# drtconway/zotmer

Measured on AMD Instinct MI355X. Metric: Gk-mers/sec kmerize k=25 on synthetic 150bp FASTQ; achieved HBM GB/s fraction, higher is better.
Workload: dtype u64

## Files before the change

### include/zotk.h

```cpp
#ifndef ZOTK_H
#define ZOTK_H

#include <stdint.h>

#ifdef __cplusplus
extern "C" {
#endif

#define ZK_OK 0
#define ZK_EINVAL (-1)
#define ZK_ENOMEM (-2)
#define ZK_EHIP (-3)
#define ZK_ENOSPC (-4)
#define ZK_EOVERFLOW (-5)
#define ZK_EINTERNAL (-6)
#define ZK_ERANGE (-7)

typedef struct zk_ctx zk_ctx;

zk_ctx* zk_create(int device, uint64_t workspace_bytes);
void zk_destroy(zk_ctx* ctx);
const char* zk_last_error(zk_ctx* ctx);
int zk_set_stream(zk_ctx* ctx, void* hip_stream);
void* zk_get_stream(zk_ctx* ctx);
// ... 8 lines not shown
int zk_copy(zk_ctx* ctx, void* d_dst, const void* d_src, uint64_t bytes);
int zk_host_alloc(zk_ctx* ctx, uint64_t bytes, void** ptr);
int zk_host_free(zk_ctx* ctx, void* ptr);
int zk_upload_async(zk_ctx* ctx, void* d_dst, const void* src, uint64_t bytes);

#define ZK_TUNE_SORT_VARIANT 1
#define ZK_TUNE_PAIRS_VARIANT 2
#define ZK_TUNE_SHORT_SORT 3
#define ZK_TUNE_XCD_GROUP 5
#define ZK_TUNE_SIDE_DIV 4
#define ZK_TUNE_EARLY_COLLAPSE 7
#define ZK_TUNE_PACKED_PAIRS 8
#define ZK_TUNE_WIDE_TILES 9
#define ZK_TUNE_STREAM_PASS 10
#define ZK_TUNE_STREAM_RANGES 11
#define ZK_TUNE_TAG_WORDS 12
#define ZK_TUNE_DEDUPE_VARIANT 13
#define ZK_TUNE_DEDUPE_LIMIT 14
#define ZK_TUNE_DEDUPE_BITS 15
#define ZK_TUNE_COMM_CHUNK 6
#define ZK_TUNE_TAG_PASS 17
#define ZK_TUNE_KWAY 18
#define ZK_TUNE_TILE_SORT 19
#define ZK_TUNE_COMM_SELF_LOOP 16
int zk_tune(zk_ctx* ctx, int what, int value);

#define ZK_PROF_HIST_STREAM 1
#define ZK_PROF_HIST_ARRAY 2
#define ZK_PROF_PASS_STREAM 3
#define ZK_PROF_PASS_KEYS 4
#define ZK_PROF_PASS_PAIRS 5
#define ZK_PROF_RLE 6
#define ZK_PROF_UNION 7
#define ZK_PROF_SELECT 8
#define ZK_PROF_MIRROR 9
#define ZK_PROF_INTERSECT 10
#define ZK_PROF_COUNT_HIST 11
#define ZK_PROF_PASS_PACKED 12
#define ZK_PROF_SAMPLE 13
#define ZK_PROF_TILE_SORT 14
#define ZK_PROF_CAPTURE_HITS 15
int zk_debug_buffer(zk_ctx* ctx, void* d_buf);
int zk_profile(zk_ctx* ctx, int enable);
int zk_profile_read(zk_ctx* ctx, int tag, uint64_t* launches, double* total_ms, uint64_t* algorithmic_bytes);


// ... 156 lines not shown
```

### zotmer_amd/csrc/context.hip

```cpp
#include <stdarg.h>
#include <string.h>

#include "internal.hpp"
#include <vector>

namespace zk {

int fail(zk_ctx* c, int code, const char* fmt, ...) {
    char buf[512];
    va_list ap;
    va_start(ap, fmt);
    vsnprintf(buf, sizeof buf, fmt, ap);
    va_end(ap);
    if (c) c->last_error = buf;
    return code;
}

void arena_reset(zk_ctx* c) { c->arena_off = 0; }

int arena_alloc(zk_ctx* c, uint64_t bytes, void** p) {
    const uint64_t need = (bytes + 255) & ~255ull;
    if (c->arena_off + need > c->arena_size) {
        if (c->arena_off != 0)
            return fail(c, ZK_ENOMEM, "workspace too small: %llu bytes in use, %llu more needed, %llu reserved (call zk_reserve)",
// ... 273 lines not shown
    if (what == ZK_TUNE_PAIRS_VARIANT) { c->pairs_variant = value; return ZK_OK; }
    if (what == ZK_TUNE_SHORT_SORT) { c->short_sort = value; return ZK_OK; }
    if (what == ZK_TUNE_SIDE_DIV) { c->side_div = value; return ZK_OK; }
    if (what == ZK_TUNE_WIDE_TILES) { c->wide_tiles = value ? 1 : 0; return ZK_OK; }
    if (what == ZK_TUNE_PACKED_PAIRS) { c->packed_pairs = value ? 1 : 0; return ZK_OK; }
    if (what == ZK_TUNE_EARLY_COLLAPSE) { c->early_collapse = value < 0 ? 0 : (value > 3 ? 3 : value); return ZK_OK; }
    if (what == ZK_TUNE_COMM_SELF_LOOP) { c->comm_self_loop = value ? 1 : 0; return ZK_OK; }
    if (what == ZK_TUNE_COMM_CHUNK) { c->comm_chunk_bytes = value > 0 ? (uint64_t)value : 0; return ZK_OK; }
    if (what == ZK_TUNE_STREAM_PASS) {
#ifdef ZK_PHASES
        c->stream_pass = value < 0 ? 0 : value;
#else
        if (value < 0 || value > 3) return fail(c, ZK_EINVAL, "stream pass variant %d (0, 1, 2 or 3)", value);
        c->stream_pass = value;
#endif
        return ZK_OK;
    }
    if (what == ZK_TUNE_TAG_WORDS) { c->tag_words = value < 0 ? 0 : (value > 2 ? 2 : value); return ZK_OK; }
    if (what == ZK_TUNE_DEDUPE_VARIANT) { c->dedupe_variant = value < 0 ? -1 : (value & 3); return ZK_OK; }
    if (what == ZK_TUNE_KWAY) { c->kway = value < 0 ? 0 : (value > 2 ? 2 : value); return ZK_OK; }
    if (what == ZK_TUNE_TILE_SORT) { c->tile_sort = value ? 1 : 0; return ZK_OK; }
    if (what == ZK_TUNE_TAG_PASS) { c->tag_pass = value ? 1 : 0; return ZK_OK; }
    if (what == ZK_TUNE_DEDUPE_BITS) { c->dedupe_bits = value < 0 ? 0 : value; return ZK_OK; }
    if (what == ZK_TUNE_DEDUPE_LIMIT) { c->dedupe_limit = value < 1 ? 1 : (value > 65536 ? 65536 : value); return ZK_OK; }
    if (what == ZK_TUNE_STREAM_RANGES) { c->stream_ranges = value < 0 ? 0 : (value > 4096 ? 4096 : value); return ZK_OK; }
    if (what == ZK_TUNE_XCD_GROUP) {
        if (value < 0 || value > 32 || (value & (value - 1))) return fail(c, ZK_EINVAL, "xcd group must be 0 or a power of two <= 32");
        c->xcd_group = value;
        return ZK_OK;
    }
    return fail(c, ZK_EINVAL, "unknown tuning knob %d", what);
}

int zk_debug_buffer(zk_ctx* c, void* d_buf) {
    if (!c) return ZK_EINVAL;
    enter(c);
    c->dbg = (u64*)d_buf;
    return ZK_OK;
}

int zk_profile(zk_ctx* c, int enable) {
    if (!c) return ZK_EINVAL;
    enter(c);
    ZK_HIP(c, hipStreamSynchronize(c->stream));
    for (auto& r : c->prof) { (void)hipEventDestroy(r.a); (void)hipEventDestroy(r.b); }
    c->prof.clear();
// ... 91 lines not shown
```

### zotmer_amd/csrc/internal.hpp

```cpp
#pragma once
#include <hip/hip_runtime.h>
#include <stdint.h>
#include <stdio.h>
#include <string>
#include <vector>

#include "../../include/zotk.h"
#include "common.hpp"

struct zk_ctx {
    int device = 0;
    hipStream_t stream = nullptr;
    bool own_stream = false;
    int num_cus = 256;
    int sort_variant = 3;
    int short_sort = 0;
    int packed_pairs = 1;
    int wide_tiles = 1;
    int early_collapse = 1;
    int side_div = 8;
    int pairs_variant = 7;
    int stream_pass = 1;
    int tag_words = 2;
    int dedupe_variant = 0;
    int dedupe_limit = 65536;
    int tag_pass = 0;
    int kway = 1;
    int tile_sort = 1;
    int dedupe_bits = 0;
    int stream_ranges = 0;

    char* arena = nullptr;
    uint64_t arena_size = 0;
    uint64_t arena_off = 0;

    char* aux = nullptr;
    uint64_t aux_size = 0;

    u64* status = nullptr;
    uint64_t status_words = 0;
    unsigned short* part16 = nullptr;
    uint64_t part16_words = 0;
    u32 epoch = 0;
    u32* d_ticket = nullptr;
    u32* d_xticket = nullptr;
    int num_xcd = 1;
    int xcd_group = 0;
    u32 ticket_base = 0;

    u32* d_err = nullptr;
    u64* d_scalars = nullptr;
    u64* h_scalars = nullptr;
// ... 63 lines not shown
struct StreamSample { int shift; uint64_t value; double max_ratio; uint64_t seen = 0, distinct = 0; bool want_distinct = false; };
struct StreamTags { bool written = false; u64* cuts = nullptr; uint32_t blocks = 0; };
struct StreamSrc { const u8* stream; uint64_t n_bytes; int K; int mode; int lo_bit; int hi_bit = 0; StreamSample* sample = nullptr;
                   StreamTags* tags = nullptr; };
int sort_rbits(zk_ctx* c);
PassPlan sort_plan_upper(zk_ctx* c, int key_bits, int lo_bit);
struct MirrorHist { int passes; int shift[4]; int bits[4]; u64* raw; };
int sort_first_bits(zk_ctx* c, int key_bits, int lo_bit);
struct DedupeResult {
    uint64_t n_out = 0;
    uint32_t flags = 0;
    uint32_t n_big = 0;
    u64 *cuts = nullptr, *nwords = nullptr, *incl = nullptr, *big = nullptr, *work = nullptr;
    u32* sub = nullptr;
    uint32_t chunks = 0;
    int pack = 0;
};
int dedupe_pass(zk_ctx* c, const u64* keys, uint64_t n, int key_bits, int b, int pack, u64* work, uint64_t cap, DedupeResult* r,
                uint64_t* n_in = nullptr, uint64_t max_chunks = 0, const u32* tags = nullptr, const u64* tag_cuts = nullptr);
int expand_tags(zk_ctx* c, const u32* tags, const u64* cuts, uint32_t blocks, int tag_bits, u64* keys_out, uint64_t first_block = 0, uint64_t n_blocks = 0);
int dedupe_finish(zk_ctx* c, const DedupeResult& r, u64* out_k, u32* out_c, u64* out_m = nullptr, int K = 0, int gbases = 0,
                  u64** mirror_hist = nullptr, int* mirror_group_bits = nullptr, bool packed_out = false);
int sort_keys_upper_counted(zk_ctx* c, u64* keys, u64* alt, uint64_t n, int key_bits, int lo_bit, u64* counted, u64** result);
int collapse_pass(zk_ctx* c, const u64* keys, uint64_t n, int shift, int bits, int pack, u64* out, uint64_t cap, uint64_t* n_out,
                  uint64_t max_tiles = 0);
int sort_stream(zk_ctx* c, const StreamSrc& src, u64* buf_a, u64* buf_b, uint64_t cap, uint64_t* n_keys,
                uint64_t acgt[4], u64** result);
struct StreamRows { u32* rows = nullptr; u64* offs = nullptr; u32 ranges = 0, radix = 0; u32* gcodes = nullptr; u16* gvalid = nullptr;
                    u32 strands = 1;
                    bool wide = false; };
int stream_hist(zk_ctx* c, const u8* stream, uint64_t n_bytes, int K, int mode, const PassPlan& plan, u64* ghist, u32 gstride,
                u64* d_acgt, u64* d_n, u64* rec_info, u64* sample, u32 sample_cap, int sample_shift, u64 sample_value, u32* sample_n,
                void* image_room, uint64_t image_room_bytes, StreamRows* out);
struct StreamPlanes { u16* dig; int shift, bits; };
int stream_pass0(zk_ctx* c, uint64_t n_bytes, int K, int mode, int shift, int bits, const u64* ghist0, const StreamRows& rows,
                 uint64_t first_nl, bool uniform, u64* kout, uint64_t n, int variant, const StreamPlanes* planes = nullptr);
int stream_pass1(zk_ctx* c, const u32* tags, const u16* dig, uint64_t n, const u64* ghist0, uint32_t radix0, int bits1, u32* tout, u64* cuts);
int tile_sort_top_bits(uint64_t n, int key_bits, int rbits);
int tile_sort(zk_ctx* c, u64* keys, u32* vals, uint64_t n, int key_bits, int top, bool* declined);
int tile_sort_count(zk_ctx* c, const u64* keys, uint64_t n, int key_bits, int top, u64* uniq, u32* counts, uint64_t cap, uint64_t* n_unique,
                    bool* declined);
int trim(zk_ctx* c, const u64* keys, const void* cnts, int cbits, uint64_t n, u64 lo, u64 hi, u64* ok, void* oc,
         uint64_t cap, uint64_t* n_out);
int project_dedupe(zk_ctx* c, const u64* keys, uint64_t n, int shift, u64* out, uint64_t cap, uint64_t* n_out);
int subsample(zk_ctx* c, const u64* keys, uint64_t n, u64 seed, double p, u64* out, uint64_t cap, uint64_t* n_out);
int sample_pairs(zk_ctx* c, const u64* keys, const u64* cnts, uint64_t n, u64 seed, double p, u64* ok, u64* oc, uint64_t cap,
// ... 38 lines not shown
```

### zotmer_amd/csrc/pipeline.hip

```cpp
#include <string.h>

#include <vector>

#include "internal.hpp"

namespace zk {

__global__ void mirror_kernel(const u64* __restrict__ c, const u32* __restrict__ n, u64 m, int K, u64* __restrict__ r,
                              u32* __restrict__ v) {
    for (u64 i = (u64)blockIdx.x * blockDim.x + threadIdx.x; i < m; i += (u64)gridDim.x * blockDim.x) {
        r[i] = revcomp(K, c[i]);
        v[i] = n[i];
    }
}

constexpr int MIRROR_GROUP_BITS = 18;
constexpr int MIRROR_GROUP_BASES = MIRROR_GROUP_BITS / 2;

__global__ void mirror_bounds_kernel(const u64* __restrict__ c, u64 n, int K, int gbits, u64* __restrict__ start) {
    const u32 g = blockIdx.x * blockDim.x + threadIdx.x;
    if (g > (1u << gbits)) return;
    const u64 want = (u64)g << (2 * K - gbits);
    u64 lo = 0, hi = n;
    if (g == (1u << gbits)) lo = n;
// ... 298 lines not shown
    u64* other = (sorted == buf_a) ? buf_b : buf_a;
    u32* cnt = (u32*)other;
    uint64_t uc = 0;
    bool in_aux = false;
    uint64_t max_count = 0;
    bool have_max = false;
    bool canon_packed = false;
    u64 *mwords = nullptr, *malt = nullptr;
    u64* mhist = nullptr;
    int mgroup = MIRROR_GROUP_BITS;
    if (dedupe_bit && n) {
        const int pk = pack_bits_for(K);
        DedupeResult r;
        uint64_t n_in = 0;
        bool done = false;
        const uint64_t nblocks = 1ull << dedupe_bit, per = n / nblocks + 1;
        const u32* tg = stags.written ? (const u32*)sorted : nullptr;
        if (!presampled) ZK_TRY(dedupe_pass(c, sorted, n, 2 * K, dedupe_bit, pk, other, cap_keys, &r, &n_in, (1u << 20) / per + 4, tg, stags.cuts));
        if (presampled || (!(r.flags & 1) && (double)r.n_out <= 0.6 * (double)n_in)) {
            ZK_TRY(dedupe_pass(c, sorted, n, 2 * K, dedupe_bit, pk, other, cap_keys, &r, nullptr, 0, tg, stags.cuts));
            if (!(r.flags & 1)) {
                uc = r.n_out;
                const uint64_t a8 = (8 * uc + 255) & ~255ull, a4 = (4 * uc + 255) & ~255ull;
                char* aux;
                ZK_TRY(aux_require(c, a8 + a4, &aux));
                const bool want_m = !(r.flags & 2) && !canonical_only && c->packed_pairs && dedupe_bit == MIRROR_GROUP_BITS &&
                                    2 * K >= MIRROR_GROUP_BITS + 8;
                ZK_TRY(dedupe_finish(c, r, (u64*)aux, (u32*)(aux + a8), want_m ? sorted : nullptr, K, MIRROR_GROUP_BASES, &mhist, &mgroup, want_m));
                if (want_m) { mwords = sorted; malt = other; canon_packed = true; }
                sorted = (u64*)aux; cnt = (u32*)(aux + a8);
                in_aux = true;
                if (!(r.flags & 2)) { max_count = (1ull << pk) - 1; have_max = true; }
                done = true;
            }
        }
        if (!done) {
            u64* res = nullptr;
            if (tg) {
                ZK_TRY(expand_tags(c, tg, stags.cuts, stags.blocks, 2 * K - dedupe_bit, other));
                u64* t = sorted; sorted = other; other = t;
            }
            ZK_TRY(sort_keys(c, sorted, other, n, 2 * K, &res));
            sorted = res;
            other = (sorted == buf_a) ? buf_b : buf_a;
            cnt = (u32*)other;
        }
        fused_bit = 0;
        collapse_bit = 0;
    }
    if (fused_bit && n) {
// ... 302 lines not shown
```

### zotmer_amd/csrc/tilesort.hip

```cpp
#include "internal.hpp"

#ifdef ZK_PHASES
#define TS_PHASE(k) do { if (a.dbg) { const u32 now__ = (u32)__builtin_amdgcn_s_memtime(); ph[k] += now__ - tlast; tlast = now__; } } while (0)
#else
#define TS_PHASE(k) do { } while (0)
#endif

namespace zk {

constexpr int TS_BLOCK = 512;
constexpr u32 TS_SLACK = 1024;

template <int ITEMS, int GROUPS, bool PAIRS>
struct TileSortSmem {
    static constexpr int CAP = TS_BLOCK * ITEMS;
    alignas(16) u64 keys[CAP];
    u32 vals[PAIRS ? CAP : 1];
    u16 idx[PAIRS ? CAP : 1];
    alignas(16) u32 start[GROUPS + 8];
    u32 wsum[TS_BLOCK / 64];
};
typedef TileSortSmem<14, 4096, false> TileSortKeys;
constexpr int TS_COUNT_ITEMS = 12;
typedef TileSortSmem<10, 2048, true> TileSortPairs;

struct TileSortArgs {
    const u64* kin; u64* kout;
    const u32* vin; u32* vout;
    const u64* bounds;
    u32 tiles;
    int pshift;
};

__global__ void tile_bounds_kernel(const u64* __restrict__ a, u64 n, int pshift, u32 T, u32 S, u32 tiles, u64* __restrict__ bounds,
                                   u32* __restrict__ flag) {
    const u32 t = blockIdx.x * blockDim.x + threadIdx.x;
    if (t > tiles) return;
    if (t == 0) { bounds[0] = 0; return; }
    if (t == tiles) { bounds[tiles] = n; return; }
    const u64 p = (u64)t * T;
    const u64 pre = a[p] >> pshift;
    u64 lo = p - S, hi = p;
    if ((a[lo] >> pshift) == pre) {
        atomicOr(flag, 1u);
        bounds[t] = lo;
        return;
    }
    while (hi - lo > 1) {
        const u64 mid = lo + (hi - lo) / 2;
        if ((a[mid] >> pshift) == pre) hi = mid; else lo = mid;
    }
    bounds[t] = hi;
}

struct TileMap {
    u64 kmin; int sh; u32 scale;
    __device__ __forceinline__ u32 group(u64 key) const {
        const u32 d = (u32)((key - kmin) >> sh);
        return scale ? __umulhi(d, scale) : d;
    }
};

template <int ITEMS, int G, bool PAIRS, class S>
__device__ __forceinline__ TileMap tile_group(S& sm, const u64* kin, const u32* vin, u64 lo, u32 m, int pshift, int tid) {
    constexpr int NW = TS_BLOCK / 64, QPT = G / TS_BLOCK / 4;
    static_assert(QPT == 1 || QPT == 2, "four or eight groups a thread in the scan");
    static_assert(S::CAP <= 8192 && G <= 4096, "group | place << 12 in a word");
    const int lane = tid & 63, wave = __builtin_amdgcn_readfirstlane(tid >> 6);
    const u64* kp = kin + lo;
    u64 k[ITEMS];
    u32 v[PAIRS ? ITEMS : 1];
#pragma unroll
    for (int j = 0; j < ITEMS; j++) {
        const u32 i = (u32)j * TS_BLOCK + tid;
        k[j] = i < m ? kp[i] : ~0ull;
        if constexpr (PAIRS) v[j] = i < m ? vin[lo + i] : 0u;
    }
    const u64 first = kp[0], last = kp[m - 1];
    TileMap tm;
    tm.kmin = (first >> pshift) << pshift;
    const u64 rm1 = (((last >> pshift) - (first >> pshift)) << pshift) | ((1ull << pshift) - 1ull);
    tm.sh = rm1 >> 32 ? 32 - __builtin_clzll(rm1) : 0;
    const u32 rs = (u32)(rm1 >> tm.sh);
    tm.scale = rs < (u32)G ? 0u : (u32)(((u64)G << 32) / ((u64)rs + 1ull));
    {
        uint4* z = reinterpret_cast<uint4*>(sm.start);
#pragma unroll
        for (int q = 0; q < QPT; q++) z[QPT * tid + q] = make_uint4(0, 0, 0, 0);
    }
    __syncthreads();
    u32 gp[ITEMS];
#pragma unroll
    for (int j = 0; j < ITEMS; j++) {
        const u32 i = (u32)j * TS_BLOCK + tid;
        const u32 g = i < m ? tm.group(k[j]) : 0u;
        gp[j] = g;
        if (i < m) gp[j] |= atomicAdd(&sm.start[g], 1u) << 12;
    }
    __syncthreads();
    {
        uint4* z = reinterpret_cast<uint4*>(sm.start);
        uint4 cq[QPT];
        u32 sum = 0;
#pragma unroll
        for (int q = 0; q < QPT; q++) { cq[q] = z[QPT * tid + q]; sum += cq[q].x + cq[q].y + cq[q].z + cq[q].w; }
        const u32 inc = wave_incl_scan_u32(sum);
        if (lane == 63) sm.wsum[wave] = inc;
        __syncthreads();
        u32 run = inc - sum;
#pragma unroll
        for (int w = 0; w < NW; w++) run += w < wave ? sm.wsum[w] : 0u;
#pragma unroll
        for (int q = 0; q < QPT; q++) {
            uint4 sq;
            sq.x = run; run += cq[q].x; sq.y = run; run += cq[q].y; sq.z = run; run += cq[q].z; sq.w = run; run += cq[q].w;
            z[QPT * tid + q] = sq;
        }
        if (tid == 0) sm.start[G] = m;
    }
    __syncthreads();
#pragma unroll
    for (int j = 0; j < ITEMS; j++) {
        const u32 i = (u32)j * TS_BLOCK + tid;
        if (i < m) {
            const u32 p = sm.start[gp[j] & (G - 1)] + (gp[j] >> 12);
            sm.keys[p] = k[j];
            if constexpr (PAIRS) { sm.vals[p] = v[j]; sm.idx[p] = (u16)i; }
        }
    }
    __syncthreads();
    return tm;
}

template <int E, bool PAIRS, class S>
__device__ __forceinline__ void tile_rank(const S& sm, const TileMap& tm, const u32 (&i)[E], u32 m, u64 (&mine)[E], u32 (&place)[E]) {
    constexpr u32 CAP = S::CAP;
    auto before = [&](u64 ko, u32 q, u64 km, u32 at) -> bool {
        if (ko != km) return ko < km;
        if constexpr (PAIRS) return q != at && sm.idx[q] < sm.idx[at];
        else return q < at;
    };
    u32 g0[E], g1[E];
#pragma unroll
    for (int e = 0; e < E; e++) mine[e] = sm.keys[i[e] < m ? i[e] : 0u];
#pragma unroll
    for (int e = 0; e < E; e++) {
        const u32 g = tm.group(mine[e]);
        g0[e] = sm.start[g]; g1[e] = sm.start[g + 1];
    }
    u64 o[E][4];
#pragma unroll
    for (int e = 0; e < E; e++)
#pragma unroll
        for (int r = 0; r < 4; r++) o[e][r] = sm.keys[g0[e] + r < CAP ? g0[e] + r : CAP - 1];
#pragma unroll
    for (int e = 0; e < E; e++) {
        const u32 at = i[e] < m ? i[e] : 0u;
        u32 rank = 0;
#pragma unroll
        for (int r = 0; r < 4; r++) {
            const u32 q = g0[e] + r;
            rank += (q < g1[e] && before(o[e][r], q, mine[e], at)) ? 1u : 0u;
        }
        for (u32 q0 = g0[e] + 4; q0 < g1[e]; q0 += 4) {
            u64 p4[4];
#pragma unroll
            for (int r = 0; r < 4; r++) p4[r] = sm.keys[q0 + r < CAP ? q0 + r : CAP - 1];
#pragma unroll
            for (int r = 0; r < 4; r++) {
                const u32 q = q0 + r;
                rank += (q < g1[e] && before(p4[r], q, mine[e], at)) ? 1u : 0u;
            }
        }
        place[e] = g0[e] + rank;
    }
}

template <int ITEMS, int G, bool PAIRS>
__global__ __launch_bounds__(TS_BLOCK, 2 * TS_BLOCK / 256) void tile_sort_kernel(TileSortArgs a) {
    using S = TileSortSmem<ITEMS, G, PAIRS>;
    constexpr int CAP = S::CAP;
    static_assert(sizeof(S) <= 80 * 1024, "two workgroups per CU");
    __shared__ S sm;
    for (u32 t = blockIdx.x; t < a.tiles; t += gridDim.x) {
        int tid = threadIdx.x;
        asm volatile("" : "+v"(tid));
        const u64 lo = a.bounds[t], hi = a.bounds[t + 1];
        if (hi - lo > (u64)CAP || hi == lo) continue;
        const u32 m = (u32)(hi - lo);
        const TileMap tm = tile_group<ITEMS, G, PAIRS>(sm, a.kin, a.vin, lo, m, a.pshift, tid);
        constexpr int E = 2;
        u64* op = a.kout + lo;
        for (u32 i0 = (u32)tid; i0 < m; i0 += E * TS_BLOCK) {
            u32 i[E], place[E];
            u64 mine[E];
#pragma unroll
            for (int e = 0; e < E; e++) i[e] = i0 + e * TS_BLOCK;
            tile_rank<E, PAIRS>(sm, tm, i, m, mine, place);
// ... 223 lines not shown
```

### zotmer_amd/native.py

```python
import ctypes as C
import os

import numpy as np

_HERE = os.path.dirname(os.path.abspath(__file__))
LIB_PATH = os.environ.get("ZOTK_LIB") or os.path.join(_HERE, "libzotk.so")

ZK_OK, ZK_EINVAL, ZK_ENOMEM, ZK_EHIP, ZK_ENOSPC, ZK_EOVERFLOW, ZK_EINTERNAL, ZK_ERANGE = 0, -1, -2, -3, -4, -5, -6, -7
KMERIZE_CANONICAL, KMERIZE_BOTH, KMERIZE_SUBSAMPLE, KMERIZE_CANONICAL_ONLY = 0, 1, 2, 4
DEFAULT_TAG_WORDS = 2

_ERRNAMES = {-1: "ZK_EINVAL", -2: "ZK_ENOMEM", -3: "ZK_EHIP", -4: "ZK_ENOSPC", -5: "ZK_EOVERFLOW",
             -6: "ZK_EINTERNAL", -7: "ZK_ERANGE"}


class ZotkError(RuntimeError):
    def __init__(self, code, msg):
        super().__init__("%s: %s" % (_ERRNAMES.get(code, code), msg))
        self.code = code


class KmerizeStats(C.Structure):
    _fields_ = [("n_windows", C.c_uint64), ("n_instances", C.c_uint64), ("n_unique", C.c_uint64),
                ("n_canonical", C.c_uint64), ("acgt", C.c_uint64 * 4)]
# ... 275 lines not shown
        cut = C.c_uint64(0)
        self._check(self.lib.zk_last_newline(self.h, text.ptr, int(n), C.byref(cut)))
        return cut.value

    def device_to_file(self, arr, fileno, offset, threads=None):
        self._check(self.lib.zk_device_to_file(self.h, arr.ptr, arr.nbytes, int(fileno), int(offset), threads or self.IO_THREADS))

    def file_to_device(self, fileno, offset, nbytes, dtype=np.uint8, threads=None):
        dt = np.dtype(dtype)
        out = self.empty(nbytes // dt.itemsize, dt)
        self._check(self.lib.zk_file_to_device(self.h, int(fileno), int(offset), int(nbytes), out.ptr, threads or self.IO_THREADS))
        return out

    def upload_stream(self, data):
        a = np.frombuffer(data, dtype=np.uint8) if isinstance(data, (bytes, bytearray, memoryview)) else np.asarray(data, np.uint8)
        return self.upload(a)

    PROF_TAGS = {"hist_stream": 1, "hist_array": 2, "pass_stream": 3, "pass_keys": 4, "pass_pairs": 5, "rle": 6,
                 "union_sum": 7, "select": 8, "mirror": 9, "intersect": 10, "count_hist": 11, "pass_packed": 12, "sample": 13, "tile_sort": 14,
                 "capture_hits": 15}

    def tune(self, sort_variant=None, pairs_variant=None, short_sort=None, side_div=None, xcd_group=None, comm_chunk=None,
             early_collapse=None, packed_pairs=None, wide_tiles=None, stream_pass=None, stream_ranges=None, tag_words=None,
             dedupe_variant=None, dedupe_limit=None, dedupe_bits=None, comm_self_loop=None, tag_pass=None, kway=None, tile_sort=None):
        if tile_sort is not None:
            self._check(self.lib.zk_tune(self.h, 19, int(tile_sort)))
        if kway is not None:
            self._check(self.lib.zk_tune(self.h, 18, int(kway)))
        if tag_pass is not None:
            self._check(self.lib.zk_tune(self.h, 17, int(tag_pass)))
        if comm_self_loop is not None:
            self._check(self.lib.zk_tune(self.h, 16, int(comm_self_loop)))
        if dedupe_bits is not None:
            self._check(self.lib.zk_tune(self.h, 15, int(dedupe_bits)))
        if dedupe_variant is not None:
            self._check(self.lib.zk_tune(self.h, 13, int(dedupe_variant)))
        if dedupe_limit is not None:
            self._check(self.lib.zk_tune(self.h, 14, int(dedupe_limit)))
        if tag_words is not None:
            self._check(self.lib.zk_tune(self.h, 12, int(tag_words)))
        if stream_pass is not None:
            self._check(self.lib.zk_tune(self.h, 10, int(stream_pass)))
        if stream_ranges is not None:
            self._check(self.lib.zk_tune(self.h, 11, int(stream_ranges)))
        if wide_tiles is not None:
            self._check(self.lib.zk_tune(self.h, 9, int(wide_tiles)))
        if packed_pairs is not None:
# ... 389 lines not shown
```

Measured before the change: 155.7.

## Merge canonical and mirrored strands per top-bit block via shared-memory tile union

For odd K with mirror output, a new path builds the reverse-complement mirror words, sorts them by their upper bits, and then merges each of the 2^18 canonical blocks with its matching mirror range inside shared memory. It writes the final keys and counts directly, which is meant to replace the dedupe_finish plus separate union pass. Blocks that are too large or too crowded go to a slower split kernel, and if that also fails the code falls back to the old path. The tile grouping code moves into a shared header so both the tile sort and this new path can use it.

```diff
diff --git a/include/zotk.h b/include/zotk.h
--- a/include/zotk.h
+++ b/include/zotk.h
@@ -54,6 +54,7 @@
 #define ZK_TUNE_TAG_PASS 17
 #define ZK_TUNE_KWAY 18
 #define ZK_TUNE_TILE_SORT 19
+#define ZK_TUNE_STRAND_BLOCKS 20
 #define ZK_TUNE_COMM_SELF_LOOP 16
 int zk_tune(zk_ctx* ctx, int what, int value);
 
diff --git a/zotmer_amd/csrc/context.hip b/zotmer_amd/csrc/context.hip
--- a/zotmer_amd/csrc/context.hip
+++ b/zotmer_amd/csrc/context.hip
@@ -319,6 +319,7 @@
     if (what == ZK_TUNE_TILE_SORT) { c->tile_sort = value ? 1 : 0; return ZK_OK; }
     if (what == ZK_TUNE_TAG_PASS) { c->tag_pass = value ? 1 : 0; return ZK_OK; }
     if (what == ZK_TUNE_DEDUPE_BITS) { c->dedupe_bits = value < 0 ? 0 : value; return ZK_OK; }
+    if (what == ZK_TUNE_STRAND_BLOCKS) { c->strand_blocks = value ? 1 : 0; return ZK_OK; }
     if (what == ZK_TUNE_DEDUPE_LIMIT) { c->dedupe_limit = value < 1 ? 1 : (value > 65536 ? 65536 : value); return ZK_OK; }
     if (what == ZK_TUNE_STREAM_RANGES) { c->stream_ranges = value < 0 ? 0 : (value > 4096 ? 4096 : value); return ZK_OK; }
     if (what == ZK_TUNE_XCD_GROUP) {
diff --git a/zotmer_amd/csrc/internal.hpp b/zotmer_amd/csrc/internal.hpp
--- a/zotmer_amd/csrc/internal.hpp
+++ b/zotmer_amd/csrc/internal.hpp
@@ -28,6 +28,7 @@
     int kway = 1;
     int tile_sort = 1;
     int dedupe_bits = 0;
+    int strand_blocks = 1;
     int stream_ranges = 0;
 
     char* arena = nullptr;
@@ -137,6 +138,8 @@
 int dedupe_finish(zk_ctx* c, const DedupeResult& r, u64* out_k, u32* out_c, u64* out_m = nullptr, int K = 0, int gbases = 0,
                   u64** mirror_hist = nullptr, int* mirror_group_bits = nullptr, bool packed_out = false);
 int sort_keys_upper_counted(zk_ctx* c, u64* keys, u64* alt, uint64_t n, int key_bits, int lo_bit, u64* counted, u64** result);
+int strand_blocks(zk_ctx* c, const DedupeResult& r, u64* keys_buf, uint64_t buf_words, int K, u64* out_k, u32* out_c, uint64_t cap,
+                  uint64_t* n_out);
 int collapse_pass(zk_ctx* c, const u64* keys, uint64_t n, int shift, int bits, int pack, u64* out, uint64_t cap, uint64_t* n_out,
                   uint64_t max_tiles = 0);
 int sort_stream(zk_ctx* c, const StreamSrc& src, u64* buf_a, u64* buf_b, uint64_t cap, uint64_t* n_keys,
diff --git a/zotmer_amd/csrc/pipeline.hip b/zotmer_amd/csrc/pipeline.hip
--- a/zotmer_amd/csrc/pipeline.hip
+++ b/zotmer_amd/csrc/pipeline.hip
@@ -344,10 +344,14 @@
             if (!(r.flags & 1)) {
                 uc = r.n_out;
                 const uint64_t a8 = (8 * uc + 255) & ~255ull, a4 = (4 * uc + 255) & ~255ull;
+                const bool want_m = !(r.flags & 2) && !canonical_only && c->packed_pairs && dedupe_bit == MIRROR_GROUP_BITS &&
+                                    2 * K >= MIRROR_GROUP_BITS + 8;
+                if (want_m && (K & 1) && c->strand_blocks && 2 * a8 <= 8 * cap_keys) {
+                    st->n_canonical = uc;
+                    return strand_blocks(c, r, sorted, cap_keys, K, out_k, out_c, cap, n_out);
+                }
                 char* aux;
                 ZK_TRY(aux_require(c, a8 + a4, &aux));
-                const bool want_m = !(r.flags & 2) && !canonical_only && c->packed_pairs && dedupe_bit == MIRROR_GROUP_BITS &&
-                                    2 * K >= MIRROR_GROUP_BITS + 8;
                 ZK_TRY(dedupe_finish(c, r, (u64*)aux, (u32*)(aux + a8), want_m ? sorted : nullptr, K, MIRROR_GROUP_BASES, &mhist, &mgroup, want_m));
                 if (want_m) { mwords = sorted; malt = other; canon_packed = true; }
                 sorted = (u64*)aux; cnt = (u32*)(aux + a8);
diff --git a/zotmer_amd/csrc/strand_blocks.hip b/zotmer_amd/csrc/strand_blocks.hip
--- /dev/null
+++ b/zotmer_amd/csrc/strand_blocks.hip
@@ -0,0 +1,314 @@
+#include "tile_group.hpp"
+
+namespace zk {
+
+constexpr int SB_ITEMS = 16, SB_GROUPS = 2048;
+constexpr u32 SB_GROUP_MAX = 128;
+typedef TileSortSmem<SB_ITEMS, SB_GROUPS, false> StrandSmem;
+constexpr int SB_BLOCK_BITS = 18;
+
+__global__ __launch_bounds__(256) void strand_mirror_kernel(const u64* __restrict__ in, const u64* __restrict__ cuts, const u64* __restrict__ incl,
+                                                            const u64* __restrict__ nwords, u32 chunks, int pack, int K, u64* __restrict__ out_m,
+                                                            MirrorHist mh) {
+    __shared__ u32 bins[4 * 512];
+    const bool hist = mh.passes > 0;
+    if (hist) {
+        for (int q = threadIdx.x; q < 4 * 512; q += blockDim.x) bins[q] = 0;
+        __syncthreads();
+    }
+    const u64 maxc = (1ull << pack) - 1;
+    for (u32 v = blockIdx.x; v < chunks; v += gridDim.x) {
+        const u64 cnt = nwords[v];
+        const u64 dst0 = incl[v] - cnt;
+        const u64* src = in + cuts[v];
+        for (u64 i0 = threadIdx.x; i0 < cnt; i0 += 4ull * blockDim.x) {
+            u64 w4[4];
+#pragma unroll
+            for (int q = 0; q < 4; q++) {
+                const u64 i = i0 + (u64)q * blockDim.x;
+                w4[q] = i < cnt ? src[i] : 0;
+            }
+#pragma unroll
+            for (int q = 0; q < 4; q++) {
+                const u64 i = i0 + (u64)q * blockDim.x;
+                if (i >= cnt) break;
+                const u64 mw = (revcomp(K, w4[q] >> pack) << pack) | (w4[q] & maxc);
+                out_m[dst0 + i] = mw;
+                if (hist) {
+#pragma unroll
+                    for (int p = 0; p < 4; p++)
+                        if (p < mh.passes) atomicAdd(&bins[p * 512 + ((u32)(mw >> mh.shift[p]) & ((1u << mh.bits[p]) - 1u))], 1u);
+                }
+            }
+        }
+    }
+    if (hist) {
+        __syncthreads();
+        for (int q = threadIdx.x; q < mh.passes * 512; q += blockDim.x)
+            if (bins[q]) atomicAdd(&mh.raw[q], (u64)bins[q]);
+    }
+}
+
+__global__ void strand_starts_kernel(const u64* __restrict__ m, u64 n, int shift, u64* __restrict__ start) {
+    const u32 g = blockIdx.x * blockDim.x + threadIdx.x;
+    if (g > (1u << SB_BLOCK_BITS)) return;
+    u64 lo = 0, hi = n;
+    if (g == (1u << SB_BLOCK_BITS)) lo = n;
+    while (lo < hi) {
+        const u64 mid = (lo + hi) >> 1;
+        if ((m[mid] >> shift) < (u64)g) lo = mid + 1; else hi = mid;
+    }
+    start[g] = lo;
+}
+
+struct StrandArgs {
+    const u64* cw;
+    const u64* cuts; const u64* nwords; const u64* incl;
+    const u64* m;
+    const u64* mstart;
+    u64* ok; u32* oc;
+    int pack;
+    int pshift;
+    u32* n_declined;
+    u32* declined;
+};
+
+__device__ __forceinline__ bool strand_crowded(const StrandSmem& sm, int tid) {
+    static_assert(SB_GROUPS == 4 * TS_BLOCK, "four groups a thread");
+    u32 big = 0;
+#pragma unroll
+    for (int q = 0; q < 4; q++) big |= sm.start[4 * tid + q + 1] - sm.start[4 * tid + q] > SB_GROUP_MAX ? 1u : 0u;
+    return __syncthreads_or((int)big) != 0;
+}
+
+__device__ __forceinline__ void strand_write(const StrandSmem& sm, const TileMap& tm, u32 m, u64* ok, u32* oc, int pack, int tid) {
+    const u64 maxc = (1ull << pack) - 1;
+    constexpr int E = 2;
+    for (u32 i0 = (u32)tid; i0 < m; i0 += E * TS_BLOCK) {
+        u32 i[E], place[E];
+        u64 mine[E];
+#pragma unroll
+        for (int e = 0; e < E; e++) i[e] = i0 + e * TS_BLOCK;
+        tile_rank<E, false>(sm, tm, i, m, mine, place);
+#pragma unroll
+        for (int e = 0; e < E; e++) {
+            if (i[e] >= m) break;
+            ok[place[e]] = mine[e] >> pack;
+            oc[place[e]] = (u32)(mine[e] & maxc);
+        }
+    }
+}
+
+__global__ __launch_bounds__(TS_BLOCK, 2 * TS_BLOCK / 256) void strand_block_union_kernel(StrandArgs a) {
+    using S = StrandSmem;
+    constexpr u32 CAP = S::CAP;
+    static_assert(sizeof(S) <= 80 * 1024, "two workgroups per CU");
+    __shared__ S sm;
+    const u32 b = blockIdx.x;
+    const u64 nc = a.nwords[b], m0 = a.mstart[b], nm = a.mstart[b + 1] - m0;
+    const u64 n = nc + nm;
+    if (n == 0) return;
+    if (n > CAP) {
+        if (threadIdx.x == 0) a.declined[atomicAdd(a.n_declined, 1u)] = b;
+        return;
+    }
+    int tid = threadIdx.x;
+    asm volatile("" : "+v"(tid));
+    const u32 m = (u32)n;
+    const TileMap tm = tile_group<SB_ITEMS, SB_GROUPS, false>(sm, a.cw, nullptr, a.cuts[b], m, a.pshift, tid, a.m, m0, (u32)nc);
+    if (strand_crowded(sm, tid)) {
+        if (tid == 0) a.declined[atomicAdd(a.n_declined, 1u)] = b;
+        return;
+    }
+    const u64 out0 = a.incl[b] - nc + m0;
+    strand_write(sm, tm, m, a.ok + out0, a.oc + out0, a.pack, tid);
+}
+
+constexpr int SB_SPLIT = 256;
+struct StrandBigSmem {
+    StrandSmem t;
+    u64 sp[SB_SPLIT];
+    u32 mcnt[SB_SPLIT + 2];
+    u32 cpos[SB_SPLIT + 2];
+    u32 tile[SB_SPLIT + 2];
+    u32 ntiles, gcount, fail;
+};
+
+__global__ __launch_bounds__(TS_BLOCK) void strand_big_block_kernel(StrandArgs a, u32 n_list, u64* __restrict__ scratch, u32* __restrict__ fail) {
+    using S = StrandBigSmem;
+    constexpr u32 CAP = StrandSmem::CAP, R = SB_SPLIT + 1;
+    __shared__ S sm;
+    u64* gat = scratch + (u64)blockIdx.x * CAP;
+    const int lane = threadIdx.x & 63;
+    for (u32 li = blockIdx.x; li < n_list; li += gridDim.x) {
+        int tid = threadIdx.x;
+        asm volatile("" : "+v"(tid));
+        const u32 b = a.declined[li];
+        const u64 nc = a.nwords[b], m0 = a.mstart[b], nm = a.mstart[b + 1] - m0;
+        const u64* C = a.cw + a.cuts[b];
+        const u64* M = a.m + m0;
+        const u64 bmin = (u64)b << a.pshift, bmax = bmin | ((1ull << a.pshift) - 1ull);
+        const u64 out0 = a.incl[b] - nc + m0;
+        u64* cand = sm.t.keys;
+        if (tid < SB_SPLIT) {
+            const bool one = nm == 0 || nc == 0;
+            const bool fromc = nm == 0 || (nc && tid < SB_SPLIT / 2);
+            const u32 j = one || fromc ? (u32)tid : (u32)tid - SB_SPLIT / 2, per = one ? SB_SPLIT : SB_SPLIT / 2;
+            cand[tid] = fromc ? C[(u64)j * nc / per] : M[(u64)j * nm / per];
+        }
+        if (tid == 0) { sm.fail = 0; sm.gcount = 0; }
+        if (tid < (int)R + 1) sm.mcnt[tid] = 0;
+        __syncthreads();
+        if (tid < SB_SPLIT) {
+            const u64 v = cand[tid];
+            u32 r = 0;
+            for (int q = 0; q < SB_SPLIT; q++) { const u64 o = cand[q]; r += (o < v || (o == v && q < tid)) ? 1u : 0u; }
+            sm.sp[r] = v;
+        }
+        __syncthreads();
+        auto range_of = [&](u64 v) -> u32 {
+            u32 lo = 0, hi = SB_SPLIT;
+            while (lo < hi) { const u32 mid = (lo + hi) >> 1; if (sm.sp[mid] <= v) lo = mid + 1; else hi = mid; }
+            return lo;
+        };
+        for (u64 i = tid; i < nm; i += TS_BLOCK) atomicAdd(&sm.mcnt[range_of(M[i])], 1u);
+        if (tid <= SB_SPLIT) {
+            u32 p = 0;
+            if (tid > 0) {
+                const u64 v = sm.sp[tid - 1];
+                u64 lo = 0, hi = nc;
+                while (lo < hi) { const u64 mid = (lo + hi) >> 1; if (C[mid] < v) lo = mid + 1; else hi = mid; }
+                p = (u32)lo;
+            }
+            sm.cpos[tid] = p;
+        }
+        if (tid == 0) sm.cpos[R] = (u32)nc;
+        __syncthreads();
+        if (tid == 0) {
+            u32 acc = 0, nt = 0, mb = 0;
+            sm.tile[nt++] = 0;
+            for (u32 j = 0; j < R; j++) {
+                const u32 mc = sm.mcnt[j], tot = sm.cpos[j + 1] - sm.cpos[j] + mc;
+                if (tot > CAP) { sm.fail = 1; break; }
+                if (acc + tot > CAP) { sm.tile[nt++] = j; acc = 0; }
+                acc += tot;
+                sm.mcnt[j] = mb;
+                mb += mc;
+            }
+            sm.mcnt[R] = mb;
+            sm.tile[nt] = R;
+            sm.ntiles = nt;
+        }
+        __syncthreads();
+        if (sm.fail) {
+            if (tid == 0) atomicOr(fail, 1u);
+            continue;
+        }
+        const u32 ntiles = sm.ntiles;
+        for (u32 t = 0; t < ntiles; t++) {
+            const u32 ra = sm.tile[t], rb = sm.tile[t + 1];
+            const u64 vlo = ra == 0 ? bmin : sm.sp[ra - 1];
+            const u64 vhi = rb == R ? bmax : sm.sp[rb - 1] - 1;
+            const u32 c_lo = sm.cpos[ra], mc = sm.cpos[rb] - c_lo, mt = sm.mcnt[rb] - sm.mcnt[ra];
+            const u32 m = mc + mt;
+            if (m == 0) continue;
+            if (mt) {
+                for (u64 i0 = 0; i0 < nm; i0 += TS_BLOCK) {
+                    const u64 i = i0 + tid;
+                    const u64 v = i < nm ? M[i] : 0;
+                    const bool in = i < nm && v >= vlo && v <= vhi;
+                    const u64 bal = __ballot(in);
+                    u32 base = 0;
+                    if (lane == 0 && bal) base = atomicAdd(&sm.gcount, (u32)__popcll(bal));
+                    base = (u32)__shfl((int)base, 0, 64);
+                    if (in) gat[base + popc_below(bal)] = v;
+                }
+                __threadfence_block();
+            }
+            __syncthreads();
+            const TileMap tm = tile_group<SB_ITEMS, SB_GROUPS, false>(sm.t, C, nullptr, c_lo, m, a.pshift, tid, gat, 0, mc, true, vlo, vhi);
+            if (strand_crowded(sm.t, tid)) {
+                if (tid == 0) atomicOr(fail, 1u);
+                break;
+            }
+            const u64 o = out0 + c_lo + sm.mcnt[ra];
+            strand_write(sm.t, tm, m, a.ok + o, a.oc + o, a.pack, tid);
+            if (tid == 0) sm.gcount = 0;
+            __syncthreads();
+        }
+        __syncthreads();
+    }
+}
+
+int strand_blocks(zk_ctx* c, const DedupeResult& r, u64* keys_buf, uint64_t buf_words, int K, u64* out_k, u32* out_c, uint64_t cap,
+                  uint64_t* n_out) {
+    *n_out = 0;
+    const uint64_t uc = r.n_out;
+    if (uc == 0) return ZK_OK;
+    if (!(K & 1) || r.n_big || r.chunks != (1u << SB_BLOCK_BITS)) return fail(c, ZK_EINTERNAL, "strand_blocks: K %d, %u big counts, %u blocks", K, r.n_big, r.chunks);
+    const uint64_t a8w = ((8 * uc + 255) & ~255ull) / 8;
+    if (2 * a8w > buf_words) return fail(c, ZK_EINTERNAL, "strand_blocks: %llu words do not fit twice in %llu", (unsigned long long)uc, (unsigned long long)buf_words);
+    if (2 * uc > cap) return fail(c, ZK_ENOSPC, "output holds %llu entries, the table has %llu", (unsigned long long)cap, (unsigned long long)(2 * uc));
+    const int pk = r.pack, key_bits = 2 * K + pk, lo_bit = key_bits - SB_BLOCK_BITS;
+    u64* mw = keys_buf;
+    u64* malt = keys_buf + a8w;
+    MirrorHist mh = {};
+    if (c->sort_variant == 3) {
+        const PassPlan plan = sort_plan_upper(c, key_bits, lo_bit);
+        if (plan.passes <= 4) {
+            ZK_TRY(arena_alloc(c, sizeof(u64) * MAX_PASSES * 512, (void**)&mh.raw));
+            ZK_HIP(c, hipMemsetAsync(mh.raw, 0, sizeof(u64) * MAX_PASSES * 512, c->stream));
+            mh.passes = plan.passes;
+            for (int p = 0; p < plan.passes; p++) { mh.shift[p] = plan.shift[p]; mh.bits[p] = plan.bits[p]; }
+        }
+    }
+    prof_begin(c, ZK_PROF_SELECT, 16 * uc);
+    hipLaunchKernelGGL(strand_mirror_kernel, dim3((u32)c->num_cus * 8), dim3(256), 0, c->stream, r.work, r.cuts, r.incl, r.nwords, r.chunks, pk, K, mw, mh);
+    prof_end(c);
+    ZK_HIP(c, hipGetLastError());
+    u64* sk = nullptr;
+    if (mh.passes) ZK_TRY(sort_keys_upper_counted(c, mw, malt, uc, key_bits, lo_bit, mh.raw, &sk));
+    else ZK_TRY(sort_keys_upper(c, mw, malt, uc, key_bits, lo_bit, &sk));
+    u64* mstart;
+    u32* declined;
+    ZK_TRY(arena_alloc(c, sizeof(u64) * ((1ull << SB_BLOCK_BITS) + 1), (void**)&mstart));
+    ZK_TRY(arena_alloc(c, sizeof(u32) * r.chunks, (void**)&declined));
+    StrandArgs a = {};
+    a.cw = r.work; a.cuts = r.cuts; a.nwords = r.nwords; a.incl = r.incl; a.m = sk; a.mstart = mstart;
+    a.ok = out_k; a.oc = out_c; a.pack = pk; a.pshift = lo_bit;
+    a.n_declined = (u32*)(c->d_scalars + 9);
+    a.declined = declined;
+    u32* fail = (u32*)(c->d_scalars + 9) + 1;
+    prof_begin(c, ZK_PROF_UNION, 8 * 2 * uc + 12 * 2 * uc);
+    hipLaunchKernelGGL(strand_starts_kernel, dim3(((1u << SB_BLOCK_BITS) + 256) / 256), dim3(256), 0, c->stream, sk, (u64)uc, lo_bit, mstart);
+    ZK_HIP(c, hipMemsetAsync(c->d_scalars + 9, 0, sizeof(u64), c->stream));
+    hipLaunchKernelGGL(strand_block_union_kernel, dim3(r.chunks), dim3(TS_BLOCK), 0, c->stream, a);
+    prof_end(c);
+    ZK_HIP(c, hipGetLastError());
+    ZK_HIP(c, hipMemcpyAsync(c->h_scalars + 9, c->d_scalars + 9, sizeof(u64), hipMemcpyDeviceToHost, c->stream));
+    ZK_TRY(check_device_error(c));
+    const uint32_t n_declined = (uint32_t)c->h_scalars[9];
+    if (n_declined) {
+        const uint32_t grid = n_declined < 2u * (uint32_t)c->num_cus ? n_declined : 2u * (uint32_t)c->num_cus;
+        u64* scratch;
+        ZK_TRY(arena_alloc(c, sizeof(u64) * StrandSmem::CAP * grid, (void**)&scratch));
+        prof_begin(c, ZK_PROF_UNION, 0);
+        hipLaunchKernelGGL(strand_big_block_kernel, dim3(grid), dim3(TS_BLOCK), 0, c->stream, a, n_declined, scratch, fail);
+        prof_end(c);
+        ZK_HIP(c, hipGetLastError());
+        ZK_HIP(c, hipMemcpyAsync(c->h_scalars + 9, c->d_scalars + 9, sizeof(u64), hipMemcpyDeviceToHost, c->stream));
+        ZK_TRY(check_device_error(c));
+    }
+    if ((uint32_t)(c->h_scalars[9] >> 32) == 0) {
+        *n_out = 2 * uc;
+        return ZK_OK;
+    }
+    char* aux;
+    ZK_TRY(aux_require(c, 8 * a8w, &aux));
+    ZK_TRY(dedupe_finish(c, r, (u64*)aux, nullptr, nullptr, K, 0, nullptr, nullptr, true));
+    u64* ms = nullptr;
+    ZK_TRY(sort_keys_upper(c, sk, sk == mw ? malt : mw, uc, key_bits, pk, &ms));
+    return union_sum_packed_ab(c, (const u64*)aux, uc, ms, uc, pk, out_k, out_c, cap, n_out, true);
+}
+
+}
diff --git a/zotmer_amd/csrc/tile_group.hpp b/zotmer_amd/csrc/tile_group.hpp
--- /dev/null
+++ b/zotmer_amd/csrc/tile_group.hpp
@@ -0,0 +1,145 @@
+#pragma once
+#include "internal.hpp"
+
+namespace zk {
+
+constexpr int TS_BLOCK = 512;
+constexpr u32 TS_SLACK = 1024;
+
+template <int ITEMS, int GROUPS, bool PAIRS>
+struct TileSortSmem {
+    static constexpr int CAP = TS_BLOCK * ITEMS;
+    alignas(16) u64 keys[CAP];
+    u32 vals[PAIRS ? CAP : 1];
+    u16 idx[PAIRS ? CAP : 1];
+    alignas(16) u32 start[GROUPS + 8];
+    u32 wsum[TS_BLOCK / 64];
+};
+struct TileMap {
+    u64 kmin; int sh; u32 scale;
+    __device__ __forceinline__ u32 group(u64 key) const {
+        const u32 d = (u32)((key - kmin) >> sh);
+        return scale ? __umulhi(d, scale) : d;
+    }
+};
+
+template <int ITEMS, int G, bool PAIRS, class S>
+__device__ __forceinline__ TileMap tile_group(S& sm, const u64* kin, const u32* vin, u64 lo, u32 m, int pshift, int tid,
+                                              const u64* kin2 = nullptr, u64 lo2 = 0, u32 m1 = ~0u, bool ranged = false, u64 vlo = 0,
+                                              u64 vhi = 0) {
+    constexpr int NW = TS_BLOCK / 64, QPT = G / TS_BLOCK / 4;
+    static_assert(QPT == 1 || QPT == 2, "four or eight groups a thread in the scan");
+    static_assert(S::CAP <= 8192 && G <= 4096, "group | place << 12 in a word");
+    const int lane = tid & 63, wave = __builtin_amdgcn_readfirstlane(tid >> 6);
+    const u64* kp = kin + lo;
+    u64 k[ITEMS];
+    u32 v[PAIRS ? ITEMS : 1];
+#pragma unroll
+    for (int j = 0; j < ITEMS; j++) {
+        const u32 i = (u32)j * TS_BLOCK + tid;
+        k[j] = i < m ? (i < m1 ? kp[i] : kin2[lo2 + (i - m1)]) : ~0ull;
+        if constexpr (PAIRS) v[j] = i < m ? vin[lo + i] : 0u;
+    }
+    u64 first, last;
+    if (ranged) { first = vlo; last = vhi; pshift = 0; }
+    else { first = m1 ? kp[0] : kin2[lo2]; last = m - 1 < m1 ? kp[m - 1] : kin2[lo2 + (m - 1 - m1)]; }
+    TileMap tm;
+    tm.kmin = (first >> pshift) << pshift;
+    const u64 rm1 = (((last >> pshift) - (first >> pshift)) << pshift) | ((1ull << pshift) - 1ull);
+    tm.sh = rm1 >> 32 ? 32 - __builtin_clzll(rm1) : 0;
+    const u32 rs = (u32)(rm1 >> tm.sh);
+    tm.scale = rs < (u32)G ? 0u : (u32)(((u64)G << 32) / ((u64)rs + 1ull));
+    {
+        uint4* z = reinterpret_cast<uint4*>(sm.start);
+#pragma unroll
+        for (int q = 0; q < QPT; q++) z[QPT * tid + q] = make_uint4(0, 0, 0, 0);
+    }
+    __syncthreads();
+    u32 gp[ITEMS];
+#pragma unroll
+    for (int j = 0; j < ITEMS; j++) {
+        const u32 i = (u32)j * TS_BLOCK + tid;
+        const u32 g = i < m ? tm.group(k[j]) : 0u;
+        gp[j] = g;
+        if (i < m) gp[j] |= atomicAdd(&sm.start[g], 1u) << 12;
+    }
+    __syncthreads();
+    {
+        uint4* z = reinterpret_cast<uint4*>(sm.start);
+        uint4 cq[QPT];
+        u32 sum = 0;
+#pragma unroll
+        for (int q = 0; q < QPT; q++) { cq[q] = z[QPT * tid + q]; sum += cq[q].x + cq[q].y + cq[q].z + cq[q].w; }
+        const u32 inc = wave_incl_scan_u32(sum);
+        if (lane == 63) sm.wsum[wave] = inc;
+        __syncthreads();
+        u32 run = inc - sum;
+#pragma unroll
+        for (int w = 0; w < NW; w++) run += w < wave ? sm.wsum[w] : 0u;
+#pragma unroll
+        for (int q = 0; q < QPT; q++) {
+            uint4 sq;
+            sq.x = run; run += cq[q].x; sq.y = run; run += cq[q].y; sq.z = run; run += cq[q].z; sq.w = run; run += cq[q].w;
+            z[QPT * tid + q] = sq;
+        }
+        if (tid == 0) sm.start[G] = m;
+    }
+    __syncthreads();
+#pragma unroll
+    for (int j = 0; j < ITEMS; j++) {
+        const u32 i = (u32)j * TS_BLOCK + tid;
+        if (i < m) {
+            const u32 p = sm.start[gp[j] & (G - 1)] + (gp[j] >> 12);
+            sm.keys[p] = k[j];
+            if constexpr (PAIRS) { sm.vals[p] = v[j]; sm.idx[p] = (u16)i; }
+        }
+    }
+    __syncthreads();
+    return tm;
+}
+
+template <int E, bool PAIRS, class S>
+__device__ __forceinline__ void tile_rank(const S& sm, const TileMap& tm, const u32 (&i)[E], u32 m, u64 (&mine)[E], u32 (&place)[E]) {
+    constexpr u32 CAP = S::CAP;
+    auto before = [&](u64 ko, u32 q, u64 km, u32 at) -> bool {
+        if (ko != km) return ko < km;
+        if constexpr (PAIRS) return q != at && sm.idx[q] < sm.idx[at];
+        else return q < at;
+    };
+    u32 g0[E], g1[E];
+#pragma unroll
+    for (int e = 0; e < E; e++) mine[e] = sm.keys[i[e] < m ? i[e] : 0u];
+#pragma unroll
+    for (int e = 0; e < E; e++) {
+        const u32 g = tm.group(mine[e]);
+        g0[e] = sm.start[g]; g1[e] = sm.start[g + 1];
+    }
+    u64 o[E][4];
+#pragma unroll
+    for (int e = 0; e < E; e++)
+#pragma unroll
+        for (int r = 0; r < 4; r++) o[e][r] = sm.keys[g0[e] + r < CAP ? g0[e] + r : CAP - 1];
+#pragma unroll
+    for (int e = 0; e < E; e++) {
+        const u32 at = i[e] < m ? i[e] : 0u;
+        u32 rank = 0;
+#pragma unroll
+        for (int r = 0; r < 4; r++) {
+            const u32 q = g0[e] + r;
+            rank += (q < g1[e] && before(o[e][r], q, mine[e], at)) ? 1u : 0u;
+        }
+        for (u32 q0 = g0[e] + 4; q0 < g1[e]; q0 += 4) {
+            u64 p4[4];
+#pragma unroll
+            for (int r = 0; r < 4; r++) p4[r] = sm.keys[q0 + r < CAP ? q0 + r : CAP - 1];
+#pragma unroll
+            for (int r = 0; r < 4; r++) {
+                const u32 q = q0 + r;
+                rank += (q < g1[e] && before(p4[r], q, mine[e], at)) ? 1u : 0u;
+            }
+        }
+        place[e] = g0[e] + rank;
+    }
+}
+
+}
diff --git a/zotmer_amd/csrc/tilesort.hip b/zotmer_amd/csrc/tilesort.hip
--- a/zotmer_amd/csrc/tilesort.hip
+++ b/zotmer_amd/csrc/tilesort.hip
@@ -1,4 +1,4 @@
-#include "internal.hpp"
+#include "tile_group.hpp"
 
 #ifdef ZK_PHASES
 #define TS_PHASE(k) do { if (a.dbg) { const u32 now__ = (u32)__builtin_amdgcn_s_memtime(); ph[k] += now__ - tlast; tlast = now__; } } while (0)
@@ -8,18 +8,6 @@
 
 namespace zk {
 
-constexpr int TS_BLOCK = 512;
-constexpr u32 TS_SLACK = 1024;
-
-template <int ITEMS, int GROUPS, bool PAIRS>
-struct TileSortSmem {
-    static constexpr int CAP = TS_BLOCK * ITEMS;
-    alignas(16) u64 keys[CAP];
-    u32 vals[PAIRS ? CAP : 1];
-    u16 idx[PAIRS ? CAP : 1];
-    alignas(16) u32 start[GROUPS + 8];
-    u32 wsum[TS_BLOCK / 64];
-};
 typedef TileSortSmem<14, 4096, false> TileSortKeys;
 constexpr int TS_COUNT_ITEMS = 12;
 typedef TileSortSmem<10, 2048, true> TileSortPairs;
@@ -51,129 +39,6 @@
         if ((a[mid] >> pshift) == pre) hi = mid; else lo = mid;
     }
     bounds[t] = hi;
-}
-
-struct TileMap {
-    u64 kmin; int sh; u32 scale;
-    __device__ __forceinline__ u32 group(u64 key) const {
-        const u32 d = (u32)((key - kmin) >> sh);
-        return scale ? __umulhi(d, scale) : d;
-    }
-};
-
-template <int ITEMS, int G, bool PAIRS, class S>
-__device__ __forceinline__ TileMap tile_group(S& sm, const u64* kin, const u32* vin, u64 lo, u32 m, int pshift, int tid) {
-    constexpr int NW = TS_BLOCK / 64, QPT = G / TS_BLOCK / 4;
-    static_assert(QPT == 1 || QPT == 2, "four or eight groups a thread in the scan");
-    static_assert(S::CAP <= 8192 && G <= 4096, "group | place << 12 in a word");
-    const int lane = tid & 63, wave = __builtin_amdgcn_readfirstlane(tid >> 6);
-    const u64* kp = kin + lo;
-    u64 k[ITEMS];
-    u32 v[PAIRS ? ITEMS : 1];
-#pragma unroll
-    for (int j = 0; j < ITEMS; j++) {
-        const u32 i = (u32)j * TS_BLOCK + tid;
-        k[j] = i < m ? kp[i] : ~0ull;
-        if constexpr (PAIRS) v[j] = i < m ? vin[lo + i] : 0u;
-    }
-    const u64 first = kp[0], last = kp[m - 1];
-    TileMap tm;
-    tm.kmin = (first >> pshift) << pshift;
-    const u64 rm1 = (((last >> pshift) - (first >> pshift)) << pshift) | ((1ull << pshift) - 1ull);
-    tm.sh = rm1 >> 32 ? 32 - __builtin_clzll(rm1) : 0;
-    const u32 rs = (u32)(rm1 >> tm.sh);
-    tm.scale = rs < (u32)G ? 0u : (u32)(((u64)G << 32) / ((u64)rs + 1ull));
-    {
-        uint4* z = reinterpret_cast<uint4*>(sm.start);
-#pragma unroll
-        for (int q = 0; q < QPT; q++) z[QPT * tid + q] = make_uint4(0, 0, 0, 0);
-    }
-    __syncthreads();
-    u32 gp[ITEMS];
-#pragma unroll
-    for (int j = 0; j < ITEMS; j++) {
-        const u32 i = (u32)j * TS_BLOCK + tid;
-        const u32 g = i < m ? tm.group(k[j]) : 0u;
-        gp[j] = g;
-        if (i < m) gp[j] |= atomicAdd(&sm.start[g], 1u) << 12;
-    }
-    __syncthreads();
-    {
-        uint4* z = reinterpret_cast<uint4*>(sm.start);
-        uint4 cq[QPT];
-        u32 sum = 0;
-#pragma unroll
-        for (int q = 0; q < QPT; q++) { cq[q] = z[QPT * tid + q]; sum += cq[q].x + cq[q].y + cq[q].z + cq[q].w; }
-        const u32 inc = wave_incl_scan_u32(sum);
-        if (lane == 63) sm.wsum[wave] = inc;
-        __syncthreads();
-        u32 run = inc - sum;
-#pragma unroll
-        for (int w = 0; w < NW; w++) run += w < wave ? sm.wsum[w] : 0u;
-#pragma unroll
-        for (int q = 0; q < QPT; q++) {
-            uint4 sq;
-            sq.x = run; run += cq[q].x; sq.y = run; run += cq[q].y; sq.z = run; run += cq[q].z; sq.w = run; run += cq[q].w;
-            z[QPT * tid + q] = sq;
-        }
-        if (tid == 0) sm.start[G] = m;
-    }
-    __syncthreads();
-#pragma unroll
-    for (int j = 0; j < ITEMS; j++) {
-        const u32 i = (u32)j * TS_BLOCK + tid;
-        if (i < m) {
-            const u32 p = sm.start[gp[j] & (G - 1)] + (gp[j] >> 12);
-            sm.keys[p] = k[j];
-            if constexpr (PAIRS) { sm.vals[p] = v[j]; sm.idx[p] = (u16)i; }
-        }
-    }
-    __syncthreads();
-    return tm;
-}
-
-template <int E, bool PAIRS, class S>
-__device__ __forceinline__ void tile_rank(const S& sm, const TileMap& tm, const u32 (&i)[E], u32 m, u64 (&mine)[E], u32 (&place)[E]) {
-    constexpr u32 CAP = S::CAP;
-    auto before = [&](u64 ko, u32 q, u64 km, u32 at) -> bool {
-        if (ko != km) return ko < km;
-        if constexpr (PAIRS) return q != at && sm.idx[q] < sm.idx[at];
-        else return q < at;
-    };
-    u32 g0[E], g1[E];
-#pragma unroll
-    for (int e = 0; e < E; e++) mine[e] = sm.keys[i[e] < m ? i[e] : 0u];
-#pragma unroll
-    for (int e = 0; e < E; e++) {
-        const u32 g = tm.group(mine[e]);
-        g0[e] = sm.start[g]; g1[e] = sm.start[g + 1];
-    }
-    u64 o[E][4];
-#pragma unroll
-    for (int e = 0; e < E; e++)
-#pragma unroll
-        for (int r = 0; r < 4; r++) o[e][r] = sm.keys[g0[e] + r < CAP ? g0[e] + r : CAP - 1];
-#pragma unroll
-    for (int e = 0; e < E; e++) {
-        const u32 at = i[e] < m ? i[e] : 0u;
-        u32 rank = 0;
-#pragma unroll
-        for (int r = 0; r < 4; r++) {
-            const u32 q = g0[e] + r;
-            rank += (q < g1[e] && before(o[e][r], q, mine[e], at)) ? 1u : 0u;
-        }
-        for (u32 q0 = g0[e] + 4; q0 < g1[e]; q0 += 4) {
-            u64 p4[4];
-#pragma unroll
-            for (int r = 0; r < 4; r++) p4[r] = sm.keys[q0 + r < CAP ? q0 + r : CAP - 1];
-#pragma unroll
-            for (int r = 0; r < 4; r++) {
-                const u32 q = q0 + r;
-                rank += (q < g1[e] && before(p4[r], q, mine[e], at)) ? 1u : 0u;
-            }
-        }
-        place[e] = g0[e] + rank;
-    }
 }
 
 template <int ITEMS, int G, bool PAIRS>
diff --git a/zotmer_amd/native.py b/zotmer_amd/native.py
--- a/zotmer_amd/native.py
+++ b/zotmer_amd/native.py
@@ -321,7 +321,10 @@
 
     def tune(self, sort_variant=None, pairs_variant=None, short_sort=None, side_div=None, xcd_group=None, comm_chunk=None,
              early_collapse=None, packed_pairs=None, wide_tiles=None, stream_pass=None, stream_ranges=None, tag_words=None,
-             dedupe_variant=None, dedupe_limit=None, dedupe_bits=None, comm_self_loop=None, tag_pass=None, kway=None, tile_sort=None):
+             dedupe_variant=None, dedupe_limit=None, dedupe_bits=None, comm_self_loop=None, tag_pass=None, kway=None, tile_sort=None,
+             strand_blocks=None):
+        if strand_blocks is not None:
+            self._check(self.lib.zk_tune(self.h, 20, int(strand_blocks)))
         if tile_sort is not None:
             self._check(self.lib.zk_tune(self.h, 19, int(tile_sort)))
         if kway is not None:
```

Result: faster. 166.5, median of 6 (+6.9%).
